# okgarces/deep-successor-features-for-transfer

Measured on AMD Instinct MI355X. Metric: env steps/sec (whole node), Reacher 8-task SF-DQN at 1/2/4/8 MI355X, higher is better.
Workload: dtype fp32; 1 GPU; reacher17-all-T8-B32 (Reacher-shape |s|=17 |a|=7 d=8, psi MLP 256x2, all heads updated per env step: main_sfdqn_torch.py path); heads_per_gpu=8, heads_total=8, global_batch=32, replay=host, parallelism=single

## Files before the change

### deep-successor-features-for-transfer_amd/csrc/sfx.hip

```cpp
#include <hip/hip_ext.h>
#include <hip/hip_runtime.h>
#include <dlfcn.h>
#include <rccl/rccl.h>

#include <cmath>
#include <cstdio>
#include <cstdlib>
#include <cstring>
#include <algorithm>
#include <atomic>
#include <chrono>
#include <deque>
#include <map>
#include <random>
#include <string>
#include <functional>
#include <tuple>
#include <utility>
#include <vector>

#include "sfx_kernels.h"
#include "sfx_gpiw.h"
#include "sfx_tsf.h"
#include "sfx_phi.h"
// ... 541 lines not shown
};

int tdg_variant(const sfx_handle* h) {
  if ((h->d & 3) != 0 || h->O > TDG_ROWS_O || h->A > 128) return 0;
  const long ta = (long)h->T * h->A;
  if (h->d <= 8 && 32 * ta <= 256 * 8) return 1;
  if (h->d <= 16 && 32 * ta <= 256 * 4) return 2;
  return 0;
}

bool can_fuse_tdg(const sfx_handle* h) { return tdg_variant(h) != 0; }

struct BwdExtra {
  int inc_step = 1;
  bool fuse_v0 = false;
  int vRole = R_V;
  const float* v_x = nullptr;
  const float* v_xn = nullptr;
  bool skip_fwd = false;
  const float* ax = nullptr;
  int aM = 0, a_noskip = 0;
  bool* skip_armed = nullptr;
  std::function<bool(int li, int tail_at, const BwdArgs& A, int ntile, double bytes)> ride;
};

bool can_fuse_v0(const sfx_handle* h, int vM) { return h->L[0].K <= KFUSE && vM * h->L[0].K <= VFUSE; }
bool can_fuse_ahead(const sfx_handle* h, int vM, int aM) {
  const int K = h->L[0].K;
  return can_fuse_v0(h, vM) && ((vM * K + 3) & ~3) + 2 * aM * K <= VFUSE && (2 * aM * K) % 4 == 0;
}

int run_bwd(sfx_handle* h, int head0, int nhead, int M, const float* x0, const float* phi, const float* r,
            float* losses, const TdgSpec& td, const BwdExtra& ex = BwdExtra()) {
  const bool fuse = can_fuse_tdg(h) && ((uintptr_t)phi & 15) == 0 &&
                    (!td.xmax || 32 * h->A <= 1024);
  if (!fuse && td.xi_dst) SFX_FAIL(SFX_E_STATE, "run_bwd: maxima re-initialisation needs the fused TD launch");
  const bool armed = td.skip && (fuse ? M <= 32 : true);
  if (!fuse)
    RC(run_tdg(h, head0, nhead, td.guess, M, td.use_gpi, td.a, phi, td.gamma, td.next, td.next_stride, td.flag,
               td.xmax, td.poloff, td.dz_scale, td.prev, armed));
  BwdArgs A{};
  A.xcd = nhead > 1 ? 1 : 0;
  A.nhead = nhead;
  A.step_in_tail = fuse ? 0 : 1;
  A.tdg_use_gpi = td.use_gpi;
  A.tdg_guess = td.guess;
  A.tdg_next_stride = td.next_stride;
  A.tdg_a = td.a;
  A.tdg_gamma = td.gamma;
  A.tdg_next = td.next;
  A.tdg_xmax = td.xmax;
  A.tdg_poloff = td.poloff;
  A.flag = td.flag;
  A.flag_value = h->T;
  A.dz_scale = td.dz_scale;
  if (armed && fuse) {
    A.tdg_prev = td.prev;
    A.skip = h->skip;
    A.skipc = h->skipc;
    A.skip_v0 = ex.skip_fwd ? 1 : 0;
  }
  if (armed) {
    A.skip = h->skip;
    A.skip_v0 = ex.skip_fwd ? 1 : 0;
  }
  if (ex.skip_armed) *ex.skip_armed = armed;
  const int tail_at = fuse ? 1 : 0;
  const bool need_tail = losses || r || !fuse;
  const double tdg_bytes = 4.0 * nhead * M * ((td.use_gpi ? h->T : 1) * h->O + 2.0 * h->O + 2.0 * h->d + 4);
  A.M = M;
  A.head0 = head0;
  A.mask = h->mask;
  A.hp = h->hp_psi;
  A.hpw = h->hp_w;
  A.x0 = x0;
  A.phi = phi;
  A.r = r;
  A.train_w = r != nullptr;
  A.losses = losses;
  A.inc_step = ex.inc_step;
  auto dw_tiles = [&](int l) { return cdiv(h->L[l].N, 32) * cdiv(h->L[l].K, 64); };
  auto geo = [&](int l) {
    const LayerGeo& L = h->L[l];
    RoleGeo r{};
    r.N = L.N;
    r.K = L.K;
    r.wOff = L.wOff;
    r.bOff = L.bOff;
    r.actIn = L.actIn;
    r.xOff = l == 0 ? -1 : h->actOff[l - 1];
    r.dzOff = h->actOff[l];
    r.dzIn = l == 0 ? 0 : h->actOff[l - 1];
    return r;
  };
  auto dx_bytes = [&](int l) {
    const LayerGeo& L = h->L[l];
    return 4.0 * ((double)L.N * L.K + (double)M * L.N + 2.0 * M * L.K);
  };
  auto dw_bytes = [&](int l) {
    const LayerGeo& L = h->L[l];
    return 24.0 * ((double)L.N * L.K + L.N) + 4.0 * ((double)M * L.N + (double)M * L.K);
  };
  const bool merge = h->bwd_merge && nhead > 1 && !ex.ride && h->NL >= 3 && M <= 32 && ex.fuse_v0 &&
                     can_fuse_v0(h, M + (ex.v_xn ? 1 : 0)) && h->L[1].N <= DX_SPLIT_N;
  for (int l = h->NL - 1; l >= (merge ? 2 : 1); --l) {
    const int li = h->NL - 1 - l;
    A.tdg = fuse && li == 0 ? 1 : 0;
    A.xi_src = A.tdg ? td.xi_src : nullptr;
    A.xi_dst = A.tdg ? td.xi_dst : nullptr;
    A.xi_copy = td.xi_copy;
    A.xi_n = td.xi_n;
    const double by = nhead * (dx_bytes(l) + (l + 1 <= h->NL - 1 ? dw_bytes(l + 1) : 0.0)) + (A.tdg ? tdg_bytes : 0.0);
    A.ra = geo(l);
    A.na = cdiv(M, 32) * cdiv(h->L[l].K, 16);
    A.dxs = 1;
    if (!A.tdg && h->dxpart && h->L[l].N > DX_SPLIT_N && M <= 32 * cdiv(h->Mmax, 32) &&
        nhead <= h->T) {
      A.dxs = cdiv(h->L[l].N, DX_SPLIT_N);
      A.dxpart = h->dxpart;
      A.dxctr = h->dxctr;
      A.na *= A.dxs;
    }
    if (l + 1 <= h->NL - 1) {
      A.rb = geo(l + 1);
      A.nb = dw_tiles(l + 1);
    } else {
      A.nb = 0;
    }
    A.nc = 0;
    A.tail = li == tail_at && need_tail ? 1 : 0;
    const int ntile = A.tdg ? A.na : A.na + A.nb + A.nc + A.tail;
    const dim3 grid = A.xcd ? dim3(8 * cdiv(nhead, 8) * ntile) : dim3(ntile, nhead);
    if (A.tdg && tdg_variant(h) == 1)
      launch(h, K_BWD, by, k_bwd_tdg<2, 8>, grid, dim3(256), h->G, A);
    else if (A.tdg)
      launch(h, K_BWD, by, k_bwd_tdg<4, 4>, grid, dim3(256), h->G, A);
    else if (!(ex.ride && nhead == 1 && !A.xcd && ex.ride(li, tail_at, A, ntile, by)))
      launch(h, K_BWD, by, h->bf16 ? k_bwd<true> : k_bwd<false>, grid, dim3(256), h->G, A);
  }
  A.na = 0;
  A.dxs = 1;
  A.tdg = 0;
  A.xi_dst = nullptr;
  A.xi_src = nullptr;
  A.rb = geo(1);
  A.nb = dw_tiles(1);
  A.rc = geo(0);
  A.nc = dw_tiles(0);
  const int last = merge ? h->NL - 2 : h->NL - 1;
  A.tail = last == tail_at && need_tail ? 1 : 0;
  double by_last = nhead * (dw_bytes(1) + dw_bytes(0));
  if (merge) {
    A.merge = 1;
    A.ra = geo(1);
    A.rd = geo(2);
    A.nd = dw_tiles(2);
    by_last += nhead * (dw_bytes(2) + dx_bytes(1) - 4.0 * M * h->L[1].K - 4.0 * M * h->L[0].N);
  }
  A.fuse_v0 = ex.fuse_v0 ? 1 : 0;
  A.vM = M + (ex.v_xn ? 1 : 0);
  A.vOff = h->actOff[0];
  A.vRole = ex.vRole;
  A.act0 = h->L[0].actOut;
  A.v_x = ex.v_x;
  A.v_xn = ex.v_xn;
  A.ax = ex.fuse_v0 ? ex.ax : nullptr;
  A.aM = ex.fuse_v0 && ex.ax ? ex.aM : 0;
  A.a_noskip = ex.a_noskip;
  const int ntile = A.nb + A.nc + A.nd + A.tail;
  if (merge)
    launch(h, K_BWD, by_last, h->bf16 ? k_bwd_mg<true> : k_bwd_mg<false>, dim3(8 * cdiv(nhead, 8) * ntile), dim3(256),
           h->G, A);
  else if (!(ex.ride && nhead == 1 && !A.xcd && ex.ride(h->NL - 1, tail_at, A, ntile, by_last)))
    launch(h, K_BWD, by_last, h->bf16 ? k_bwd<true> : k_bwd<false>,
           A.xcd ? dim3(8 * cdiv(nhead, 8) * ntile) : dim3(ntile, nhead), dim3(256), h->G, A);
  LAUNCHCHK();
  return SFX_OK;
}

GpiArgs gpi_args(int role, int rowoff, int row0, const float* w, float* psi, float* q, int64_t* task, int64_t* next,
                 int64_t* sel, int select_task, int use_gpi, int M) {
  GpiArgs A{};
  A.M = M;
  A.role = role;
  A.row0 = row0;
  A.rowoff = rowoff;
  A.select_task = select_task;
  A.use_gpi = use_gpi;
  A.w = w;
  A.psi_out = psi;
  A.q_out = q;
  A.task_out = task;
  A.next_out = next;
  A.sel_out = sel;
  return A;
}

int run_gpi(sfx_handle* h, const GpiArgs& A) {
  launch(h, K_GPI, 4.0 * A.M * ((double)h->T * h->O * (A.psi_out ? 2 : 1) + h->d + (A.q_out ? h->T * h->A : 0)),
         k_gpi, dim3(A.M), dim3(256), h->G, A);
  LAUNCHCHK();
  return SFX_OK;
}

int run_ver(sfx_handle* h, int M, int npol, bool sel, int post, const GpiArgs& g, const int64_t* spec,
            bool post_host = false) {
  VerArgs V{};
  V.M = M;
  V.post = post;
  V.npol = npol;
  V.sel = sel ? 1 : 0;
  V.spec_stride = MMAX;
  V.spec_next = spec;
  V.flag = &h->dout->flag;
  V.g = g;
  const int TA = h->T * h->A;
  V.rows = TA >= 256 ? 1 : (256 / TA < M ? 256 / TA : M);
  const bool wide = wide_gpi(h) && npol > 1;
  const dim3 grid = wide ? dim3(M, cdiv(npol, WPC) + 1) : dim3(npol + 1, cdiv(M, V.rows));
  if (sel && h->pub_res && h->fold_publish) {
    V.pub = h->pub_res;
    V.pub_dctr = h->pub_dctr;
    V.done = &h->dout->done;
    V.nblocks = (int)(grid.x * grid.y);
    h->pub_folded = true;
  } else if (post_host) {
    V.h_sel = h->hout->sel;
    V.h_flag = &h->hout->flag;
    V.h_posted = &h->hout->posted;
    V.done = &h->dout->done;
    V.nblocks = (int)(grid.x * grid.y);
    h->hout_posted = true;
  }
  const double by = 4.0 * (double)M * npol * h->T * h->O + 4.0 * h->T * h->O;
  if (wide)
    launch(h, K_VER, by, SFX_WIDE(k_verw), grid, dim3(256), h->G, V);
  else
    launch(h, K_VER, by, k_ver, grid, dim3(256), h->G, V);
  LAUNCHCHK();
  return SFX_OK;
}

void after_update(sfx_handle* h, int t) {
  h->host_step[t] += 1;
  h->since_target[t] += 1;
}

int maybe_sync_target(sfx_handle* h, int t) {
  if (h->since_target[t] >= h->target_update_ev) {
    touch(h);
    HIPCHK(hipMemcpyAsync(h->target_of(t), h->online_cur(t), sizeof(float) * h->P, hipMemcpyDeviceToDevice,
                          h->stream));
    if (h->bf16)
      HIPCHK(hipMemcpyAsync(h->tg16_of(t), h->on16_cur(t), sizeof(__bf16) * h->P, hipMemcpyDeviceToDevice,
                            h->stream));
    h->since_target[t] = 0;
  }
  return SFX_OK;
}

void pack_head(const sfx_handle* h, const float* src, float* dst) {
  std::memset(dst, 0, sizeof(float) * h->P);
  size_t off = 0;
  for (const LayerGeo& L : h->L) {
    std::memcpy(dst + L.wOff, src + off, sizeof(float) * L.N * L.K);
    off += (size_t)L.N * L.K;
    std::memcpy(dst + L.bOff, src + off, sizeof(float) * L.N);
    off += L.N;
  }
}

void unpack_head(const sfx_handle* h, const float* src, float* dst) {
  size_t off = 0;
  for (const LayerGeo& L : h->L) {
    std::memcpy(dst + off, src + L.wOff, sizeof(float) * L.N * L.K);
    off += (size_t)L.N * L.K;
    std::memcpy(dst + off, src + L.bOff, sizeof(float) * L.N);
    off += L.N;
  }
}

bool valid_head(const sfx_handle* h, int t) { return h && t >= 0 && t < h->T; }
bool valid_w(const sfx_handle* h, int t) { return h && t >= 0 && t < h->Tg; }

__global__ void k_to_bf16(const float* __restrict__ src, __bf16* __restrict__ dst, long long n) {
  for (long long i = (long long)blockIdx.x * blockDim.x + threadIdx.x; i < n; i += (long long)gridDim.x * blockDim.x)
    dst[i] = (__bf16)src[i];
}

int refresh_bf16(sfx_handle* h, const float* src, __bf16* dst, long long n) {
  touch(h);
  hipLaunchKernelGGL(k_to_bf16, dim3((unsigned)std::min<long long>(1024, (n + 255) / 256)), dim3(256), 0, h->stream, src,
                     dst, n);
  LAUNCHCHK();
  return SFX_OK;
}

void free_all(sfx_handle* h) {
  clear_graphs(h);
  for (auto& r : h->prof_recs) {
    (void)hipEventDestroy(r.a);
    (void)hipEventDestroy(r.b);
  }
  for (hipEvent_t e : h->prof_pool) (void)hipEventDestroy(e);
  for (void* p : {(void*)h->online, (void*)h->target, (void*)h->am, (void*)h->av, (void*)h->w, (void*)h->wm,
                  (void*)h->wv, (void*)h->step, (void*)h->dcancel, (void*)h->adamc, (void*)h->act, (void*)h->dz, (void*)h->rowloss, (void*)h->spec_next, (void*)h->skip, (void*)h->skipc,
// ... 1167 lines not shown
```

### deep-successor-features-for-transfer_amd/csrc/sfx_kernels.h

```cpp
#pragma once
#include <hip/hip_runtime.h>
#include <stdint.h>

#include <type_traits>

namespace sfx {

typedef float floatx4 __attribute__((ext_vector_type(4)));

constexpr int NLMAX = 8;
constexpr int MT = 32;
constexpr int QMAX = 8192;
constexpr int OMAX = 4096;
constexpr int DMAX = 256;
constexpr int MMAX = 1024;
constexpr int KFUSE = 64;
constexpr int GEMV_N = 512;
constexpr int GEMV_M = 4;
constexpr int DX_SPLIT_N = 256;
constexpr int VFUSE = 4096;
constexpr int TQF = 4096;

enum { ACT_NONE = 0, ACT_RELU = 1, ACT_TANH = 2 };
enum { R_S = 0, R_S1T = 1, R_S1 = 2, R_G = 3, R_A = 4, R_V = 5, R_V2 = 6, R_NS = 7, R_NS1T = 8, R_NS1 = 9, NROLE = 10 };
// ... 1285 lines not shown
  const float* Xin = layer_input(G, A, head, L.xOff);
  float* out = G.dzp(head, L.dzIn);
  const int ma = m0 + r, mb = m0 + 16 + r, kk = k0 + r;
  const bool oka = ma < M, okb = mb < M, okk = kk < K;
  const int s = (threadIdx.x >> 6) & 1, Lx = threadIdx.x & 63, col = k0 + (Lx & 15);
  float xin[4] = {0.f, 0.f, 0.f, 0.f};
  if (threadIdx.x < 128 && col < K) {
#pragma unroll
    for (int i = 0; i < 4; ++i) {
      const int row = m0 + 16 * s + (Lx >> 4) * 4 + i;
      if (row < M) xin[i] = Xin[(size_t)row * K + col];
    }
  }
  floatx4 acc0 = {0.f, 0.f, 0.f, 0.f}, acc1 = {0.f, 0.f, 0.f, 0.f};
  if constexpr (TDG) {
    __shared__ TdgSmem sm;
    if (tile == 0 && A.inc_step && threadIdx.x == 0 && !step_cancelled(G.cancel)) {
      const int st = G.step[head] + 1;
      const AdamC ac = adam_consts(A.hp, st);
      if constexpr (C) {
        __hip_atomic_store(G.step + head, st, __ATOMIC_RELAXED, __HIP_MEMORY_SCOPE_AGENT);
        float* f = reinterpret_cast<float*>(G.adamc + head);
        stc<true>(f, ac.omb1);
        stc<true>(f + 1, ac.b2);
        stc<true>(f + 2, ac.omb2);
        stc<true>(f + 3, ac.eps);
        stc<true>(f + 4, ac.wd);
        stc<true>(f + 5, ac.bc2s);
        stc<true>(f + 6, ac.nss);
      } else {
        G.step[head] = st;
        G.adamc[head] = ac;
      }
    }
    if (A.flag && tile == 0 && head == A.head0 && threadIdx.x == 0) *A.flag = A.flag_value;
    const int wpc = N > 64 ? 2 : 4, jw = 16 / wpc, j0 = (wave % wpc) * jw;
    const int nb = (wave / wpc) * 64 + g * 16;
    float bw[16];
#pragma unroll
    for (int j = 0; j < 16; ++j)
      bw[j] = (j >= j0 && j < j0 + jw && okk && nb + j < N) ? W[(size_t)(nb + j) * K + kk] : 0.f;
    if (tdg_rows<VMAX, U, C>(G, A, head, m0, tile % ntk == 0, sm)) return;
    const float* da = sm.dz + (size_t)r * N + nb;
    const float* db = sm.dz + (size_t)(16 + r) * N + nb;
#pragma unroll
    for (int j = 0; j < 16; ++j) {
      if (j >= j0 && j < j0 + jw) {
        const bool okj = nb + j < N;
        acc0 = mfma4(oka && okj ? da[j] : 0.f, bw[j], acc0);
        acc1 = mfma4(okb && okj ? db[j] : 0.f, bw[j], acc1);
      }
    }
  } else {
    const int kks[1] = {kk};
    floatx4 acc[1][2] = {{acc0, acc1}};
    dx_accum<C, BF, 1>(G.dzp(head, L.dzOff), W, BF ? G.on16 + G.slot_off(rslot(A.mask, head), head) + L.wOff : nullptr, N, K,
                       nbeg, nend, ma, mb, oka, okb, kks, acc);
    acc0 = acc[0][0];
    acc1 = acc[0][1];
  }
  PROBE_MARK();
  red[wave][0][lane] = acc0;
  red[wave][1][lane] = acc1;
  __syncthreads();
  if (!TDG && A.dxs > 1) {
    const int ntile = ((M + 31) >> 5) * ntk;
    const size_t pt = ((size_t)(head - A.head0) * ntile + tile) * A.dxs;
    __shared__ int s_last;
    if (threadIdx.x < 128) {
      const floatx4 v = dx_red_sum(red, s, Lx);
      float* o = A.dxpart + ((pt + split) * 128 + threadIdx.x) * 4;
#ifdef SFX_CHECK
      SFX_CHK((long long)((pt + split) * 128 + threadIdx.x) * 4 + 3 < G.ext_dxpart, pt, split, G.ext_dxpart);
#endif
#pragma unroll
      for (int i = 0; i < 4; ++i) stc<true>(o + i, v[i]);
      asm volatile("s_waitcnt vmcnt(0)" ::: "memory");
    }
    __syncthreads();
    if (threadIdx.x == 0) {
      unsigned* ctr = A.dxctr + (size_t)(head - A.head0) * ntile + tile;
      const unsigned prev = __hip_atomic_fetch_add(ctr, 1u, __ATOMIC_RELAXED, __HIP_MEMORY_SCOPE_AGENT);
      s_last = prev == (unsigned)A.dxs - 1;
      if (s_last) __hip_atomic_store(ctr, 0u, __ATOMIC_RELAXED, __HIP_MEMORY_SCOPE_AGENT);
    }
    __syncthreads();
    if (!s_last || threadIdx.x >= 128) return;
    floatx4 v = {0.f, 0.f, 0.f, 0.f};
    for (int q = 0; q < A.dxs; ++q) {
      const float* o = A.dxpart + ((pt + q) * 128 + threadIdx.x) * 4;
#pragma unroll
      for (int i = 0; i < 4; ++i) v[i] = __fadd_rn(v[i], ldc<true>(o + i));
    }
    if (col < K) {
#pragma unroll
      for (int i = 0; i < 4; ++i) {
        const int row = m0 + 16 * s + (Lx >> 4) * 4 + i;
        if (row < M) {
          G.chk_act(L.dzIn, (long long)row * K + col);
          stc<C>(out + (size_t)row * K + col, act_bwd(v[i], xin[i], L.actIn));
        }
      }
    }
    return;
  }
  if (threadIdx.x < 128) {
    const floatx4 v = dx_red_sum(red, s, Lx);
    if (col < K) {
#pragma unroll
      for (int i = 0; i < 4; ++i) {
        const int row = m0 + 16 * s + (Lx >> 4) * 4 + i;
        if (row < M) {
          G.chk_act(L.dzIn, (long long)row * K + col);
          stc<C>(out + (size_t)row * K + col, act_bwd(v[i], xin[i], L.actIn));
        }
      }
    }
  }
}

__device__ __forceinline__ int v0_aoff(const BwdArgs& A, int K) { return (A.vM * K + 3) & ~3; }
constexpr int V0S = KFUSE + 4;

template <bool C>
__device__ __forceinline__ void v0_tile(const float* x, int K, int m0, int rows, const float* w, float bb, int act,
                                        float* Y, int N, int n, long long lim) {
  constexpr int KS = 8;
  const int lane = threadIdx.x & 63, r = lane & 15, g = lane >> 4, ma = m0 + r;
  floatx4 c = {0.f, 0.f, 0.f, 0.f};
  for (int k0 = 0; k0 < K; k0 += 4 * KS) {
    float a[KS], b[KS];
#pragma unroll
    for (int q = 0; q < KS; ++q) {
      const int k = k0 + 4 * q + g;
      a[q] = (k < K && ma < rows) ? x[ma * K + k] : 0.f;
      b[q] = k < K ? w[k] : 0.f;
    }
#pragma unroll
    for (int q = 0; q < KS; ++q)
      if (k0 + 4 * q < K) c = mfma4(a[q], b[q], c);
  }
  if (n < N) {
#pragma unroll
    for (int i = 0; i < 4; ++i) {
      const int m = m0 + g * 4 + i;
      if (m < rows) {
        SFX_CHK((long long)m * N + n < lim, m, n, lim);
        stc<C>(Y + (size_t)m * N + n, act_fwd(__fadd_rn(c[i], bb), act));
      }
    }
  }
}

template <bool C>
__device__ __forceinline__ void fused_v0(const Geo& G, const BwdArgs& A, const RoleGeo& L, int head, int nbase, const float* sW,
                         const float* sB, const float* sX, const float* sWt = nullptr, const float* sBt = nullptr,
                         bool vrows = true, bool landed = false) {
  if (A.aM > 0 && !landed) asm volatile("s_waitcnt vmcnt(0)" ::: "memory");
  __syncthreads();
  PROBE_AT(3);
  const int K = L.K, N = L.N, VM = A.vM;
  const int wave = threadIdx.x >> 6, lane = threadIdx.x & 63, r = lane & 15;
  const int nl = (wave & 1) * 16 + r, n = nbase + nl;
  const float bias = sB[nl];
  if (vrows) {
    float* Y = G.actp(A.vRole, head, A.vOff);
    for (int mt = wave >> 1; mt * 16 < VM; mt += 2)
      v0_tile<C>(sX, K, mt * 16, VM, sW + nl * V0S, bias, A.act0, Y, N, n, G.actSize - A.vOff);
  }
  PROBE_AT(4);
  if (A.aM > 0) {
    const int aM = A.aM, nt = (aM + 15) >> 4;
    const float* xa = sX + v0_aoff(A, K);
    const float bt = sBt[nl];
    for (int it = wave >> 1; it < 3 * nt; it += 2) {
      const int which = it / nt, mt = it - which * nt;
      v0_tile<C>(xa + (which ? aM * K : 0), K, mt * 16, aM, which == 2 ? sWt + nl * K : sW + nl * V0S,
                 which == 2 ? bt : bias, A.act0, G.actp(which == 0 ? R_NS : which == 1 ? R_NS1 : R_NS1T, head, A.vOff),
                 N, n, G.actSize - A.vOff);
    }
  }
  PROBE_AT(5);
}

typedef __attribute__((address_space(3))) void* tsf_lds_t;

template <class F>
__device__ __forceinline__ void glds(float* dst, int n, F src, int w0 = 0, int nw = 4) {
  const int lane = threadIdx.x & 63, wv = (threadIdx.x >> 6) - w0;
  if (wv < 0 || wv >= nw) return;
  for (int c = wv; c * 64 < n; c += nw) {
    const int j = c * 64 + lane;
    const float* p = j < n ? src(j) : nullptr;
    if (p)
      __builtin_amdgcn_global_load_lds((const void*)p, (tsf_lds_t)(dst + c * 64), 4, 0, 0);
    else if (j < n)
      dst[j] = 0.f;
  }
}

struct V0Smem {
  float sW[32 * V0S];
  float sB[32];
  float sWt[32 * KFUSE];
  float sBt[32];
  __align__(16) float sX[VFUSE];
};
__device__ __forceinline__ V0Smem& v0_smem() {
  __shared__ V0Smem sm;
  return sm;
}

__device__ __forceinline__ void v0_stage_ahead(const Geo& G, const BwdArgs& A, const RoleGeo& L, int head, int nbase,
                                               V0Smem& sm) {
  const int K = L.K, ncol = L.N - nbase < 32 ? L.N - nbase : 32;
  const float* ax = A.ax;
  glds(sm.sX + v0_aoff(A, K), 2 * A.aM * K, [&](int j) -> const float* { return ax + j; });
  const float* Pt = G.target + (long long)head * G.P;
  const float* tw = Pt + L.wOff + (size_t)nbase * K;
  glds(sm.sWt, 32 * K, [&](int j) -> const float* { return j < ncol * K ? tw + j : nullptr; });
  const float* tb = Pt + L.bOff + nbase;
  glds(sm.sBt, 32, [&](int j) -> const float* { return j < ncol ? tb + j : nullptr; }, 0, 1);
}

__device__ __forceinline__ void role_v0_only(const Geo& G, const BwdArgs& A, int head, const RoleGeo& L, int tile, bool vrows) {
  const int N = L.N, K = L.K, M = A.M, tid = threadIdx.x, nbase = tile * 32;
  const float* Pw = G.online + G.slot_off(rslot(A.mask, head) ^ 1, head);
  V0Smem& sm = v0_smem();
  float* sW = sm.sW;
  float* sB = sm.sB;
  float* sX = sm.sX;
  if (A.aM > 0) v0_stage_ahead(G, A, L, head, nbase, sm);
  const FDiv fK = fdiv(K);
  for (int j = tid; j < 32 * K; j += 256) {
    const int nl = j / fK, k = j - nl * K;
    sW[nl * V0S + k] = nbase + nl < N ? Pw[L.wOff + (size_t)(nbase + nl) * K + k] : 0.f;
  }
  if (tid < 32) sB[tid] = nbase + tid < N ? Pw[L.bOff + nbase + tid] : 0.f;
  if (vrows) {
    const int nxs = A.vM * K;
    for (int j = tid; j < nxs; j += 256) sX[j] = j < M * K ? A.v_x[j] : A.v_xn[j - M * K];
  }
  fused_v0<false>(G, A, L, head, nbase, sW, sB, sX, sm.sWt, sm.sBt, vrows);
}

template <bool C = false, bool BF = false, bool MG = false>
__device__ __forceinline__ void role_dw(const Geo& G, const BwdArgs& A, int head, const RoleGeo& L, int tile, bool fuse,
                                        floatx4 (*red)[2][64] = nullptr) {
  const int N = L.N, K = L.K, M = A.M;
  const int ntk = (K + 63) >> 6;
  const int kt = tile % ntk, nt = tile / ntk;
  const int wave = threadIdx.x >> 6, lane = threadIdx.x & 63, r = lane & 15, g = lane >> 4;
  const int nbase = nt * 32, n0 = nbase + (wave & 1) * 16, k0 = kt * 64 + (wave >> 1) * 32;
  const float* dZ = G.dzp(head, L.dzOff);
  const float* X = layer_input(G, A, head, L.xOff);
  const int rs = rslot(A.mask, head);
  const long long ro = G.slot_off(rs, head), wo = G.slot_off(rs ^ 1, head);
  const float* Pr = G.online + ro;
  const float* Mr = G.am + ro;
  const float* Vr = G.av + ro;
  float* Pw = G.online + wo;
  float* Mw = G.am + wo;
  float* Vw = G.av + wo;
  const AdamC c = load_adamc<C>(G.adamc + head);
  const int cx = step_cancelled(G.cancel);
  const int nn = n0 + r, kb0 = k0 + r, kb1 = k0 + 16 + r;
  float pp[8], pm[8], pv[8];
  bool ok[8];
#pragma unroll
  for (int i = 0; i < 4; ++i) {
    const int n = n0 + g * 4 + i;
#pragma unroll
    for (int h = 0; h < 2; ++h) {
      const int k = h ? kb1 : kb0;
      const int e = i * 2 + h;
      ok[e] = n < N && k < K;
      const size_t off = (size_t)L.wOff + (size_t)n * K + k;
      pp[e] = ok[e] ? Pr[off] : 0.f;
      pm[e] = ok[e] ? Mr[off] : 0.f;
      pv[e] = ok[e] ? Vr[off] : 0.f;
    }
  }
  const bool dob = kt == 0 && wave < 2 && g == 0 && nn < N;
  const int nbias = nn;
  float bp = 0.f, bm = 0.f, bv = 0.f;
  if (dob) {
    bp = Pr[L.bOff + nbias];
    bm = Mr[L.bOff + nbias];
    bv = Vr[L.bOff + nbias];
  }
  constexpr int XQ = VFUSE / 1024;
  float4 xs[XQ];
  float xn = 0.f;
  const int nx = fuse ? M * K : 0;
  const int nxn = fuse && A.v_xn ? K : 0;
  if (fuse && A.aM > 0) v0_stage_ahead(G, A, L, head, nbase, v0_smem());
  if (fuse) {
    if ((nx & 3) == 0 && (reinterpret_cast<uintptr_t>(A.v_x) & 15) == 0) {
#pragma unroll
      for (int q = 0; q < XQ; ++q) {
        const int j = threadIdx.x + 256 * q;
        xs[q] = 4 * j < nx ? reinterpret_cast<const float4*>(A.v_x)[j] : make_float4(0.f, 0.f, 0.f, 0.f);
      }
    } else {
#pragma unroll
      for (int q = 0; q < XQ; ++q) {
        const int j = 4 * (threadIdx.x + 256 * q);
        xs[q].x = j < nx ? A.v_x[j] : 0.f;
        xs[q].y = j + 1 < nx ? A.v_x[j + 1] : 0.f;
        xs[q].z = j + 2 < nx ? A.v_x[j + 2] : 0.f;
        xs[q].w = j + 3 < nx ? A.v_x[j + 3] : 0.f;
      }
    }
    if ((int)threadIdx.x < nxn) xn = A.v_xn[threadIdx.x];
  }
  __builtin_amdgcn_sched_barrier(0);
  floatx4 acc0 = {0.f, 0.f, 0.f, 0.f}, acc1 = {0.f, 0.f, 0.f, 0.f};
  float bsum = 0.f;
  float dz0[MT / 4], xb0[MT / 4], xb1[MT / 4];
  if constexpr (MG) {
    static_assert(MT == 32, "merged tile: the 32 rows of one dX tile are the one row chunk of dW");
    __shared__ floatx4 red2[4][2][64];
    const RoleGeo& L1 = A.ra;
    const float* Y0 = layer_input(G, A, head, L1.xOff);
    float y0[MT / 4];
#pragma unroll
    for (int j = 0; j < MT / 4; ++j) {
      const int m = 4 * j + g;
      y0[j] = (m < M && nn < N) ? Y0[(size_t)m * N + nn] : 0.f;
      xb0[j] = (m < M && kb0 < K) ? X[(size_t)m * K + kb0] : 0.f;
      xb1[j] = (m < M && kb1 < K) ? X[(size_t)m * K + kb1] : 0.f;
    }
    const int kks[2] = {nbase + r, nbase + 16 + r};
    floatx4 dacc[2][2] = {};
    dx_accum<false, BF, 2>(G.dzp(head, L1.dzOff), Pr + L1.wOff, BF ? G.on16 + ro + L1.wOff : nullptr, L1.N, L1.K, 0, L1.N, r,
                           16 + r, r < M, 16 + r < M, kks, dacc);
    red[wave][0][lane] = dacc[0][0];
    red[wave][1][lane] = dacc[0][1];
    red2[wave][0][lane] = dacc[1][0];
    red2[wave][1][lane] = dacc[1][1];
    PROBE_AT(6);
    __syncthreads();
    const floatx4 (*rd)[2][64] = (wave & 1) ? red2 : red;
#pragma unroll
    for (int j = 0; j < MT / 4; ++j) {
      const int s = j >> 2, Lx = (j & 3) * 16 + r;
      float v = rd[0][s][Lx][g];
      v = __fadd_rn(v, rd[1][s][Lx][g]);
      v = __fadd_rn(v, rd[2][s][Lx][g]);
      v = __fadd_rn(v, rd[3][s][Lx][g]);
      dz0[j] = (4 * j + g < M && nn < N) ? act_bwd(v, y0[j], L1.actIn) : 0.f;
    }
    PROBE_AT(7);
  }
  for (int mc = 0; mc < M; mc += MT) {
    float av[MT / 4], bv0[MT / 4], bv1[MT / 4];
#pragma unroll
    for (int j = 0; j < MT / 4; ++j) {
      const int m = mc + 4 * j + g;
      const bool okm = m < M;
      if constexpr (MG) {
        av[j] = dz0[j];
        bv0[j] = xb0[j];
        bv1[j] = xb1[j];
        continue;
      }
      av[j] = (okm && nn < N) ? ldc<C>(dZ + (size_t)m * N + nn) : 0.f;
      bv0[j] = (okm && kb0 < K) ? X[(size_t)m * K + kb0] : 0.f;
      bv1[j] = (okm && kb1 < K) ? X[(size_t)m * K + kb1] : 0.f;
    }
#pragma unroll
    for (int j = 0; j < MT / 4; ++j) {
      acc0 = mfma4(av[j], bv0[j], acc0);
      acc1 = mfma4(av[j], bv1[j], acc1);
    }
#pragma unroll
    for (int j = 0; j < MT / 4; ++j) bsum = __fadd_rn(bsum, av[j]);
  }
  bsum = __fadd_rn(bsum, __shfl_xor(bsum, 16));
  bsum = __fadd_rn(bsum, __shfl_xor(bsum, 32));
  if (fuse && A.aM > 0) asm volatile("s_waitcnt vmcnt(0)" ::: "memory");
  PROBE_MARK();
  V0Smem& sm = v0_smem();
  float* sW = sm.sW;
  float* sB = sm.sB;
  float* sX = sm.sX;
  if (fuse) {
#pragma unroll
    for (int q = 0; q < XQ; ++q) {
      const int j = threadIdx.x + 256 * q;
      if (4 * j + 3 < nx) {
        reinterpret_cast<float4*>(sX)[j] = xs[q];
      } else if (4 * j < nx) {
        sX[4 * j] = xs[q].x;
        if (4 * j + 1 < nx) sX[4 * j + 1] = xs[q].y;
        if (4 * j + 2 < nx) sX[4 * j + 2] = xs[q].z;
      }
    }
    if ((int)threadIdx.x < nxn) sX[nx + threadIdx.x] = xn;
  }
#pragma unroll
  for (int i = 0; i < 4; ++i) {
    const int n = n0 + g * 4 + i;
#pragma unroll
    for (int h = 0; h < 2; ++h) {
      const int e = i * 2 + h;
      if (ok[e]) {
        const int k = h ? kb1 : kb0;
        const size_t off = (size_t)L.wOff + (size_t)n * K + k;
        SFX_CHK((long long)off < G.P, L.wOff, n, k);
        adam_apply(pp[e], pm[e], pv[e], h ? acc1[i] : acc0[i], c);
        if (!cx) {
          st_param<C>(Pw + off, pp[e]);
          st_moment(Mw + off, pm[e]);
          st_moment(Vw + off, pv[e]);
          if constexpr (BF) G.on16[wo + off] = (__bf16)pp[e];
        }
        if (fuse) sW[(n - nbase) * V0S + k] = pp[e];
      }
    }
  }
  if (dob) {
    adam_apply(bp, bm, bv, bsum, c);
    if (!cx) {
      st_param<C>(Pw + L.bOff + nbias, bp);
      st_moment(Mw + L.bOff + nbias, bm);
      st_moment(Vw + L.bOff + nbias, bv);
      if constexpr (BF) G.on16[wo + L.bOff + nbias] = (__bf16)bp;
    }
    if (fuse) sB[nbias - nbase] = bp;
  }
  if (fuse) fused_v0<C>(G, A, L, head, nbase, sW, sB, sX, sm.sWt, sm.sBt, true, true);
}

__device__ __forceinline__ float block_sum(float v, float* red) {
  red[threadIdx.x] = v;
  __syncthreads();
#pragma unroll
  for (int s = 128; s >= 1; s >>= 1) {
    if ((int)threadIdx.x < s) red[threadIdx.x] = __fadd_rn(red[threadIdx.x], red[threadIdx.x + s]);
    __syncthreads();
  }
  const float r = red[0];
  __syncthreads();
  return r;
}

__device__ __forceinline__ void role_tail(const Geo& G, const BwdArgs& A, int head) {
  const int M = A.M, d = G.d, tid = threadIdx.x;
  __shared__ float s_e[MMAX];
  __shared__ float s_red[256];
  __shared__ float s_phi[2048];
  const int step = A.step_in_tail && A.inc_step ? G.step[head] + 1 : G.step[head];
  const int cx = step_cancelled(G.cancel);
  const float* rl = G.rowloss + (long long)head * MMAX;
  float* w = G.w + (long long)head * G.dpad;
  float part = 0.f;
  for (int b = tid; b < M; b += 256) part = __fadd_rn(part, rl[b]);
  float l2 = 0.f;
  if (A.train_w) {
    const bool lds_phi = M * d <= 2048;
    if (lds_phi)
      for (int j = tid; j < M * d; j += 256) s_phi[j] = A.phi[j];
    __syncthreads();
    const float* ph = lds_phi ? s_phi : A.phi;
    float se = 0.f;
    for (int b = tid; b < M; b += 256) {
      float rf = 0.f;
      for (int k = 0; k < d; ++k) rf = __builtin_fmaf(w[k], ph[(size_t)b * d + k], rf);
      s_e[b] = __fsub_rn(rf, A.r[b]);
      se = __builtin_fmaf(s_e[b], s_e[b], se);
    }
    se = block_sum(se, s_red);
    const AdamC c = adam_consts(A.hpw, step);
    const float nrm = (float)(2.0 / (double)M);
    float gw = 0.f;
    if (tid < d) {
      for (int b = 0; b < M; ++b) gw = __builtin_fmaf(__fmul_rn(nrm, s_e[b]), ph[(size_t)b * d + tid], gw);
    }
    __syncthreads();
    if (tid < d && !cx) adam_el(w + tid, G.wm + (long long)head * G.dpad + tid, G.wv + (long long)head * G.dpad + tid, gw, c);
    l2 = (float)((double)se / (double)M);
  }
  const float s = A.losses ? block_sum(part, s_red) : 0.f;
  if (tid == 0) {
    const float l1 = (float)((double)s / ((double)M * (double)G.O));
    if (A.losses) {
      float* lo = A.losses + 3 * (head - A.head0);
      lo[0] = __fadd_rn(l1, l2);
      lo[1] = l1;
      lo[2] = l2;
    }
    if (A.step_in_tail && !cx) {
      G.step[head] = step;
      G.adamc[head] = adam_consts(A.hp, step);
    }
  }
}

template <bool BF, bool MG = false>
__device__ __forceinline__ void bwd_body(const Geo& G, const BwdArgs& A, int head, int bx, floatx4 (*red)[2][64]) {
  PROBE_T(pt0);
  PROBE_MARKA();
  const bool skip = A.skip && __builtin_nontemporal_load(A.skip + head) != 0;
  if (bx < A.nc) {
    if (skip) {
      if (A.fuse_v0 && (!A.skip_v0 || (A.aM > 0 && A.a_noskip))) role_v0_only(G, A, head, A.rc, bx, !A.skip_v0);
      return;
    }
    role_dw<false, BF, MG>(G, A, head, A.rc, bx, A.fuse_v0 != 0, red);
    PROBE_REC(6, pt0);
    return;
  }
  bx -= A.nc;
  if (bx < A.nd) {
    if (skip) return;
    role_dw<false, BF>(G, A, head, A.rd, bx, false);
    PROBE_REC(5, pt0);
    return;
  }
  bx -= A.nd;
  if (bx < A.nb) {
    if (skip) return;
    role_dw<false, BF>(G, A, head, A.rb, bx, false);
    PROBE_REC(5, pt0);
    return;
  }
  bx -= A.nb;
  if (bx < A.na) {
    if (skip) return;
    role_dx<false, 2, 8, false, BF>(G, A, head, bx, red);
    PROBE_REC(4, pt0);
    return;
  }
  role_tail(G, A, head);
}

template <bool BF = false>
__global__ __launch_bounds__(256) void k_bwd(Geo G, BwdArgs A) {
  __shared__ floatx4 red[4][2][64];
  int head = A.head0 + blockIdx.y, bx = blockIdx.x;
  if (A.xcd) {
    if (!xcd_decode(blockIdx.x, A.nhead, A.na + A.nb + A.nc + A.nd + A.tail, head, bx)) return;
    head += A.head0;
  }
  bwd_body<BF>(G, A, head, bx, red);
}

template <bool BF = false>
__global__ __launch_bounds__(256) void k_bwd_mg(Geo G, BwdArgs A) {
  __shared__ floatx4 red[4][2][64];
  int head, bx;
  if (!xcd_decode(blockIdx.x, A.nhead, A.na + A.nb + A.nc + A.nd + A.tail, head, bx)) return;
  bwd_body<BF, true>(G, A, head + A.head0, bx, red);
}

template <int VMAX, int U>
__global__ __launch_bounds__(256) void k_bwd_tdg(Geo G, BwdArgs A) {
  __shared__ floatx4 red[4][2][64];
  PROBE_T(pt0);
  if (A.xi_dst)
    fill_sortable(A.xi_dst, A.xi_src, A.xi_copy, A.xi_n, (blockIdx.y * gridDim.x + blockIdx.x) * 256 + threadIdx.x,
                  gridDim.x * gridDim.y * 256);
  int head = A.head0 + blockIdx.y, bx = blockIdx.x;
  if (A.xcd) {
    if (!xcd_decode(blockIdx.x, A.nhead, A.na, head, bx)) return;
    head += A.head0;
  }
  PROBE_MARKA();
  role_dx<true, VMAX, U>(G, A, head, bx, red);
  PROBE_REC(3, pt0);
}

struct GpiArgs {
  int M, role, row0, select_task, use_gpi, rowoff;
  int w_stride, sel_stride;
  const float* w;
  float* psi_out;
  float* q_out;
  int64_t* task_out;
  int64_t* next_out;
  int64_t* sel_out;
  const unsigned long long* out_ind;
};

__device__ __forceinline__ unsigned long long argmax_key(float v, int idx) {
  const unsigned int u = __float_as_uint(__fadd_rn(v, 0.f));
  const unsigned int o = (u & 0x80000000u) ? ~u : (u | 0x80000000u);
  return ((unsigned long long)o << 32) | (unsigned long long)(0xFFFFFFFFu - (unsigned)idx);
}
__device__ __forceinline__ int argmax_idx(unsigned long long key) { return (int)(0xFFFFFFFFu - (unsigned)(key & 0xFFFFFFFFull)); }
__device__ __forceinline__ unsigned long long wave_max(unsigned long long k) {
#pragma unroll
  for (int m = 32; m >= 1; m >>= 1) {
    const unsigned long long o = __shfl_xor(k, m, 64);
    k = o > k ? o : k;
  }
  return k;
}

__device__ __forceinline__ int gpi_pick(const GpiArgs& A, const float* s_q, float* s_mt, float* s_ma, int T, int Aa,
                                        long long ob, int64_t* so, int nthr) {
  const int tid = threadIdx.x;
  for (int t = tid; t < T; t += nthr) {
    float mx = s_q[t * Aa];
    for (int a = 1; a < Aa; ++a) mx = fmaxf(mx, s_q[t * Aa + a]);
    s_mt[t] = mx;
  }
  for (int a = tid; a < Aa; a += nthr) {
    float mx = s_q[a];
    for (int t = 1; t < T; ++t) mx = fmaxf(mx, s_q[t * Aa + a]);
    s_ma[a] = mx;
  }
  __syncthreads();
  int picked = -1;
  if (tid < 64) {
    unsigned long long kt = 0ull, ka = 0ull;
    for (int t = tid; t < T; t += 64) {
      const unsigned long long k = argmax_key(s_mt[t], t);
      kt = k > kt ? k : kt;
    }
    for (int a = tid; a < Aa; a += 64) {
      const unsigned long long k = argmax_key(s_ma[a], a);
      ka = k > ka ? k : ka;
    }
    const int tb = argmax_idx(wave_max(kt)), ab = argmax_idx(wave_max(ka));
    const int c = A.use_gpi ? tb : A.select_task;
    unsigned long long kc = 0ull;
    if (so)
      for (int a = tid; a < Aa; a += 64) {
        const unsigned long long k = argmax_key(s_q[c * Aa + a], a);
        kc = k > kc ? k : kc;
      }
    const int act = so ? argmax_idx(wave_max(kc)) : 0;
    if (so) picked = c * Aa + act;
    if (tid == 0) {
      if (A.task_out) A.task_out[ob] = tb;
      if (A.next_out) A.next_out[ob] = ab;
      if (so) {
        __hip_atomic_store(so, (int64_t)c, __ATOMIC_RELAXED, __HIP_MEMORY_SCOPE_AGENT);
        __hip_atomic_store(so + 1, (int64_t)act, __ATOMIC_RELAXED, __HIP_MEMORY_SCOPE_AGENT);
      }
    }
  }
  return picked;
}

__device__ void gpi_row(const Geo& G, const GpiArgs& A0, int b) {
  GpiArgs A = A0;
  if (A.out_ind) {
    A.q_out = reinterpret_cast<float*>(A.out_ind[0]);
    A.task_out = reinterpret_cast<int64_t*>(A.out_ind[1]);
  }
  const int tid = threadIdx.x;
  const int T = G.T, Aa = G.A, d = G.d, O = G.O, NLm = G.lastOff, TA = T * Aa;
  __shared__ float s_q[QMAX];
  __shared__ float s_w[DMAX];
  __shared__ float s_mt[256], s_ma[256];
  const long long ob = (long long)(A.row0 + b);
  const int lb = A.rowoff + b;
// ... 794 lines not shown
```

Measured before the change: 8309 env steps/s.

## Narrow merged backward layer-0 tiles to 16 columns to double block count

In the merged last-layers backward kernel, the layer-0 weight-gradient tiles are halved from 32 to 16 output columns, so each wave covers a 16-wide k slice. The host sets the tile count to match, and the dX recompute, the LDS reduction and the fused forward recompute are templated on the tile width. The aim is more blocks for the tiny Reacher layer-0 and fewer registers and less LDS per block, giving better occupancy. The cost is that the shared dX reduction work is repeated across twice as many blocks.

```diff
diff --git a/deep-successor-features-for-transfer_amd/csrc/sfx.hip b/deep-successor-features-for-transfer_amd/csrc/sfx.hip
--- a/deep-successor-features-for-transfer_amd/csrc/sfx.hip
+++ b/deep-successor-features-for-transfer_amd/csrc/sfx.hip
@@ -717,6 +717,7 @@
   double by_last = nhead * (dw_bytes(1) + dw_bytes(0));
   if (merge) {
     A.merge = 1;
+    A.nc = cdiv(h->L[0].N, 16);
     A.ra = geo(1);
     A.rd = geo(2);
     A.nd = dw_tiles(2);
diff --git a/deep-successor-features-for-transfer_amd/csrc/sfx_kernels.h b/deep-successor-features-for-transfer_amd/csrc/sfx_kernels.h
--- a/deep-successor-features-for-transfer_amd/csrc/sfx_kernels.h
+++ b/deep-successor-features-for-transfer_amd/csrc/sfx_kernels.h
@@ -1461,7 +1461,7 @@
   }
 }
 
-template <bool C>
+template <bool C, int NW = 32>
 __device__ __forceinline__ void fused_v0(const Geo& G, const BwdArgs& A, const RoleGeo& L, int head, int nbase, const float* sW,
                          const float* sB, const float* sX, const float* sWt = nullptr, const float* sBt = nullptr,
                          bool vrows = true, bool landed = false) {
@@ -1469,12 +1469,15 @@
   __syncthreads();
   PROBE_AT(3);
   const int K = L.K, N = L.N, VM = A.vM;
+  static_assert(NW == 16 || NW == 32, "layer-0 tile width");
+  constexpr int WS = NW == 32 ? 2 : 4;
   const int wave = threadIdx.x >> 6, lane = threadIdx.x & 63, r = lane & 15;
-  const int nl = (wave & 1) * 16 + r, n = nbase + nl;
+  const int wt = NW == 32 ? wave >> 1 : wave;
+  const int nl = (NW == 32 ? (wave & 1) * 16 : 0) + r, n = nbase + nl;
   const float bias = sB[nl];
   if (vrows) {
     float* Y = G.actp(A.vRole, head, A.vOff);
-    for (int mt = wave >> 1; mt * 16 < VM; mt += 2)
+    for (int mt = wt; mt * 16 < VM; mt += WS)
       v0_tile<C>(sX, K, mt * 16, VM, sW + nl * V0S, bias, A.act0, Y, N, n, G.actSize - A.vOff);
   }
   PROBE_AT(4);
@@ -1482,7 +1485,7 @@
     const int aM = A.aM, nt = (aM + 15) >> 4;
     const float* xa = sX + v0_aoff(A, K);
     const float bt = sBt[nl];
-    for (int it = wave >> 1; it < 3 * nt; it += 2) {
+    for (int it = wt; it < 3 * nt; it += WS) {
       const int which = it / nt, mt = it - which * nt;
       v0_tile<C>(xa + (which ? aM * K : 0), K, mt * 16, aM, which == 2 ? sWt + nl * K : sW + nl * V0S,
                  which == 2 ? bt : bias, A.act0, G.actp(which == 0 ? R_NS : which == 1 ? R_NS1 : R_NS1T, head, A.vOff),
@@ -1508,59 +1511,66 @@
   }
 }
 
+template <int NW = 32>
 struct V0Smem {
-  float sW[32 * V0S];
-  float sB[32];
-  float sWt[32 * KFUSE];
-  float sBt[32];
+  float sW[NW * V0S];
+  float sB[NW];
+  float sWt[NW * KFUSE];
+  float sBt[NW];
   __align__(16) float sX[VFUSE];
 };
-__device__ __forceinline__ V0Smem& v0_smem() {
-  __shared__ V0Smem sm;
+template <int NW = 32>
+__device__ __forceinline__ V0Smem<NW>& v0_smem() {
+  __shared__ V0Smem<NW> sm;
   return sm;
 }
 
+template <int NW>
 __device__ __forceinline__ void v0_stage_ahead(const Geo& G, const BwdArgs& A, const RoleGeo& L, int head, int nbase,
-                                               V0Smem& sm) {
-  const int K = L.K, ncol = L.N - nbase < 32 ? L.N - nbase : 32;
+                                               V0Smem<NW>& sm) {
+  const int K = L.K, ncol = L.N - nbase < NW ? L.N - nbase : NW;
   const float* ax = A.ax;
   glds(sm.sX + v0_aoff(A, K), 2 * A.aM * K, [&](int j) -> const float* { return ax + j; });
   const float* Pt = G.target + (long long)head * G.P;
   const float* tw = Pt + L.wOff + (size_t)nbase * K;
-  glds(sm.sWt, 32 * K, [&](int j) -> const float* { return j < ncol * K ? tw + j : nullptr; });
+  glds(sm.sWt, NW * K, [&](int j) -> const float* { return j < ncol * K ? tw + j : nullptr; });
   const float* tb = Pt + L.bOff + nbase;
-  glds(sm.sBt, 32, [&](int j) -> const float* { return j < ncol ? tb + j : nullptr; }, 0, 1);
-}
-
+  glds(sm.sBt, NW, [&](int j) -> const float* { return j < ncol ? tb + j : nullptr; }, 0, 1);
+}
+
+template <int NW = 32>
 __device__ __forceinline__ void role_v0_only(const Geo& G, const BwdArgs& A, int head, const RoleGeo& L, int tile, bool vrows) {
-  const int N = L.N, K = L.K, M = A.M, tid = threadIdx.x, nbase = tile * 32;
+  const int N = L.N, K = L.K, M = A.M, tid = threadIdx.x, nbase = tile * NW;
   const float* Pw = G.online + G.slot_off(rslot(A.mask, head) ^ 1, head);
-  V0Smem& sm = v0_smem();
+  V0Smem<NW>& sm = v0_smem<NW>();
   float* sW = sm.sW;
   float* sB = sm.sB;
   float* sX = sm.sX;
   if (A.aM > 0) v0_stage_ahead(G, A, L, head, nbase, sm);
   const FDiv fK = fdiv(K);
-  for (int j = tid; j < 32 * K; j += 256) {
+  for (int j = tid; j < NW * K; j += 256) {
     const int nl = j / fK, k = j - nl * K;
     sW[nl * V0S + k] = nbase + nl < N ? Pw[L.wOff + (size_t)(nbase + nl) * K + k] : 0.f;
   }
-  if (tid < 32) sB[tid] = nbase + tid < N ? Pw[L.bOff + nbase + tid] : 0.f;
+  if (tid < NW) sB[tid] = nbase + tid < N ? Pw[L.bOff + nbase + tid] : 0.f;
   if (vrows) {
     const int nxs = A.vM * K;
     for (int j = tid; j < nxs; j += 256) sX[j] = j < M * K ? A.v_x[j] : A.v_xn[j - M * K];
   }
-  fused_v0<false>(G, A, L, head, nbase, sW, sB, sX, sm.sWt, sm.sBt, vrows);
+  fused_v0<false, NW>(G, A, L, head, nbase, sW, sB, sX, sm.sWt, sm.sBt, vrows);
 }
 
 template <bool C = false, bool BF = false, bool MG = false>
 __device__ __forceinline__ void role_dw(const Geo& G, const BwdArgs& A, int head, const RoleGeo& L, int tile, bool fuse,
                                         floatx4 (*red)[2][64] = nullptr) {
+  constexpr int NW = MG ? 16 : 32;
+  constexpr int NH = MG ? 1 : 2;
   const int N = L.N, K = L.K, M = A.M;
   const int ntk = (K + 63) >> 6;
   const int kt = tile % ntk, nt = tile / ntk;
   const int wave = threadIdx.x >> 6, lane = threadIdx.x & 63, r = lane & 15, g = lane >> 4;
-  const int nbase = nt * 32, n0 = nbase + (wave & 1) * 16, k0 = kt * 64 + (wave >> 1) * 32;
+  const int nbase = nt * NW, n0 = MG ? nbase : nbase + (wave & 1) * 16;
+  const int k0 = kt * 64 + (MG ? wave * 16 : (wave >> 1) * 32);
   const float* dZ = G.dzp(head, L.dzOff);
   const float* X = layer_input(G, A, head, L.xOff);
   const int rs = rslot(A.mask, head);
@@ -1574,15 +1584,15 @@
   const AdamC c = load_adamc<C>(G.adamc + head);
   const int cx = step_cancelled(G.cancel);
   const int nn = n0 + r, kb0 = k0 + r, kb1 = k0 + 16 + r;
-  float pp[8], pm[8], pv[8];
-  bool ok[8];
+  float pp[4 * NH], pm[4 * NH], pv[4 * NH];
+  bool ok[4 * NH];
 #pragma unroll
   for (int i = 0; i < 4; ++i) {
     const int n = n0 + g * 4 + i;
 #pragma unroll
-    for (int h = 0; h < 2; ++h) {
+    for (int h = 0; h < NH; ++h) {
       const int k = h ? kb1 : kb0;
-      const int e = i * 2 + h;
+      const int e = i * NH + h;
       ok[e] = n < N && k < K;
       const size_t off = (size_t)L.wOff + (size_t)n * K + k;
       pp[e] = ok[e] ? Pr[off] : 0.f;
@@ -1590,7 +1600,7 @@
       pv[e] = ok[e] ? Vr[off] : 0.f;
     }
   }
-  const bool dob = kt == 0 && wave < 2 && g == 0 && nn < N;
+  const bool dob = kt == 0 && wave < (MG ? 1 : 2) && g == 0 && nn < N;
   const int nbias = nn;
   float bp = 0.f, bm = 0.f, bv = 0.f;
   if (dob) {
@@ -1603,7 +1613,7 @@
   float xn = 0.f;
   const int nx = fuse ? M * K : 0;
   const int nxn = fuse && A.v_xn ? K : 0;
-  if (fuse && A.aM > 0) v0_stage_ahead(G, A, L, head, nbase, v0_smem());
+  if (fuse && A.aM > 0) v0_stage_ahead(G, A, L, head, nbase, v0_smem<NW>());
   if (fuse) {
     if ((nx & 3) == 0 && (reinterpret_cast<uintptr_t>(A.v_x) & 15) == 0) {
 #pragma unroll
@@ -1626,10 +1636,9 @@
   __builtin_amdgcn_sched_barrier(0);
   floatx4 acc0 = {0.f, 0.f, 0.f, 0.f}, acc1 = {0.f, 0.f, 0.f, 0.f};
   float bsum = 0.f;
-  float dz0[MT / 4], xb0[MT / 4], xb1[MT / 4];
+  float dz0[MT / 4], xb0[MT / 4];
   if constexpr (MG) {
     static_assert(MT == 32, "merged tile: the 32 rows of one dX tile are the one row chunk of dW");
-    __shared__ floatx4 red2[4][2][64];
     const RoleGeo& L1 = A.ra;
     const float* Y0 = layer_input(G, A, head, L1.xOff);
     float y0[MT / 4];
@@ -1638,26 +1647,22 @@
       const int m = 4 * j + g;
       y0[j] = (m < M && nn < N) ? Y0[(size_t)m * N + nn] : 0.f;
       xb0[j] = (m < M && kb0 < K) ? X[(size_t)m * K + kb0] : 0.f;
-      xb1[j] = (m < M && kb1 < K) ? X[(size_t)m * K + kb1] : 0.f;
-    }
-    const int kks[2] = {nbase + r, nbase + 16 + r};
-    floatx4 dacc[2][2] = {};
-    dx_accum<false, BF, 2>(G.dzp(head, L1.dzOff), Pr + L1.wOff, BF ? G.on16 + ro + L1.wOff : nullptr, L1.N, L1.K, 0, L1.N, r,
+    }
+    const int kks[1] = {nbase + r};
+    floatx4 dacc[1][2] = {};
+    dx_accum<false, BF, 1>(G.dzp(head, L1.dzOff), Pr + L1.wOff, BF ? G.on16 + ro + L1.wOff : nullptr, L1.N, L1.K, 0, L1.N, r,
                            16 + r, r < M, 16 + r < M, kks, dacc);
     red[wave][0][lane] = dacc[0][0];
     red[wave][1][lane] = dacc[0][1];
-    red2[wave][0][lane] = dacc[1][0];
-    red2[wave][1][lane] = dacc[1][1];
     PROBE_AT(6);
     __syncthreads();
-    const floatx4 (*rd)[2][64] = (wave & 1) ? red2 : red;
 #pragma unroll
     for (int j = 0; j < MT / 4; ++j) {
       const int s = j >> 2, Lx = (j & 3) * 16 + r;
-      float v = rd[0][s][Lx][g];
-      v = __fadd_rn(v, rd[1][s][Lx][g]);
-      v = __fadd_rn(v, rd[2][s][Lx][g]);
-      v = __fadd_rn(v, rd[3][s][Lx][g]);
+      float v = red[0][s][Lx][g];
+      v = __fadd_rn(v, red[1][s][Lx][g]);
+      v = __fadd_rn(v, red[2][s][Lx][g]);
+      v = __fadd_rn(v, red[3][s][Lx][g]);
       dz0[j] = (4 * j + g < M && nn < N) ? act_bwd(v, y0[j], L1.actIn) : 0.f;
     }
     PROBE_AT(7);
@@ -1671,7 +1676,6 @@
       if constexpr (MG) {
         av[j] = dz0[j];
         bv0[j] = xb0[j];
-        bv1[j] = xb1[j];
         continue;
       }
       av[j] = (okm && nn < N) ? ldc<C>(dZ + (size_t)m * N + nn) : 0.f;
@@ -1681,7 +1685,7 @@
 #pragma unroll
     for (int j = 0; j < MT / 4; ++j) {
       acc0 = mfma4(av[j], bv0[j], acc0);
-      acc1 = mfma4(av[j], bv1[j], acc1);
+      if constexpr (!MG) acc1 = mfma4(av[j], bv1[j], acc1);
     }
 #pragma unroll
     for (int j = 0; j < MT / 4; ++j) bsum = __fadd_rn(bsum, av[j]);
@@ -1690,7 +1694,7 @@
   bsum = __fadd_rn(bsum, __shfl_xor(bsum, 32));
   if (fuse && A.aM > 0) asm volatile("s_waitcnt vmcnt(0)" ::: "memory");
   PROBE_MARK();
-  V0Smem& sm = v0_smem();
+  V0Smem<NW>& sm = v0_smem<NW>();
   float* sW = sm.sW;
   float* sB = sm.sB;
   float* sX = sm.sX;
@@ -1712,8 +1716,8 @@
   for (int i = 0; i < 4; ++i) {
     const int n = n0 + g * 4 + i;
 #pragma unroll
-    for (int h = 0; h < 2; ++h) {
-      const int e = i * 2 + h;
+    for (int h = 0; h < NH; ++h) {
+      const int e = i * NH + h;
       if (ok[e]) {
         const int k = h ? kb1 : kb0;
         const size_t off = (size_t)L.wOff + (size_t)n * K + k;
@@ -1739,7 +1743,7 @@
     }
     if (fuse) sB[nbias - nbase] = bp;
   }
-  if (fuse) fused_v0<C>(G, A, L, head, nbase, sW, sB, sX, sm.sWt, sm.sBt, true, true);
+  if (fuse) fused_v0<C, NW>(G, A, L, head, nbase, sW, sB, sX, sm.sWt, sm.sBt, true, true);
 }
 
 __device__ __forceinline__ float block_sum(float v, float* red) {
@@ -1814,7 +1818,7 @@
   const bool skip = A.skip && __builtin_nontemporal_load(A.skip + head) != 0;
   if (bx < A.nc) {
     if (skip) {
-      if (A.fuse_v0 && (!A.skip_v0 || (A.aM > 0 && A.a_noskip))) role_v0_only(G, A, head, A.rc, bx, !A.skip_v0);
+      if (A.fuse_v0 && (!A.skip_v0 || (A.aM > 0 && A.a_noskip))) role_v0_only<MG ? 16 : 32>(G, A, head, A.rc, bx, !A.skip_v0);
       return;
     }
     role_dw<false, BF, MG>(G, A, head, A.rc, bx, A.fuse_v0 != 0, red);
```

Measured after the change: 8771 env steps/s (median of 6 runs). 1.06x the previous value.
